# cvg/nice-slam

Measured on AMD Instinct MI355X. Metric: rendered rays/sec (fwd+bwd) per mapping iter, higher is better.
Workload: dtype f32 (f64 sample placement / depth)

## Files before the change

### include/nsr.h

```cpp
#ifndef NSR_H_
#define NSR_H_

#include <stdint.h>

#ifdef __cplusplus
extern "C" {
#endif

#define NSR_VERSION 8

enum { NSR_STAGE_COARSE = 0, NSR_STAGE_MIDDLE = 1, NSR_STAGE_FINE = 2, NSR_STAGE_COLOR = 3 };
enum { NSR_COARSE = 0, NSR_MIDDLE = 1, NSR_FINE = 2, NSR_COLOR = 3 };

#define NSR_MAX_SAMPLES 64

typedef struct nsr_grid {
    const float *feat;
    float *dfeat;
    int32_t Z, Y, X;
    int32_t pad_;
    double lo[3];
    double hi[3];
} nsr_grid;

// ... 43 lines not shown
    const double *d_depth;
    const double *d_var;
    const float *d_rgb;
    const double *depth;
    float *d_rays_o;
    float *d_rays_d;
    float *workspace;
    int64_t workspace_floats;
    int32_t max_blocks;
    int32_t overwrite_dparams;
    void *ev_start;
    void *ev_stop;
    const double *grad_scale;
    int32_t loss_grads_from_forward;
    int32_t pad_;
    void *ev_dx_done;
    void *ev_dw_done;
} nsr_bwd_args;

int nsr_version(void);
const char *nsr_last_error(void);

int64_t nsr_param_count(int slot);
int64_t nsr_packed_count(int slot);
int64_t nsr_acts_floats(int stage, int64_t n_rays, int n_samples_total);

int64_t nsr_bwd_workspace_floats(int stage, int64_t n_rays, int n_samples_total, int max_blocks);

int nsr_pack_params(int slot, const float *params, float *packed, void *stream);

int nsr_render_fwd(const nsr_render_args *a, void *stream);
int nsr_render_bwd(const nsr_render_args *a, const nsr_bwd_args *b, void *stream);

int nsr_eval_points_fwd(const nsr_render_args *a, const double *points, int64_t n_points, float *out, void *stream);

int nsr_get_samples(const int64_t *indices, int64_t n, int32_t H0, int32_t H1, int32_t W0, int32_t W1,
                    int32_t W_full, float fx, float fy, float cx, float cy,
                    const float *c2w, int32_t c2w_stride, const float *depth, const float *color,
                    float *rays_o, float *rays_d, float *out_depth, float *out_color, void *stream);

typedef struct nsr_frame {
    const float *depth;
    const float *color;
    const float *c2w;
    int32_t c2w_stride;
    int32_t pad_;
} nsr_frame;
int nsr_get_samples_window(const int64_t *indices, int32_t K, int64_t n, int32_t H0, int32_t H1, int32_t W0, int32_t W1,
                           int32_t W_full, float fx, float fy, float cx, float cy, const nsr_frame *frames,
                           float *rays_o, float *rays_d, float *out_depth, float *out_color,
                           const double *bound_lo, const double *bound_hi, uint8_t *keep, float *kept_max, void *stream);
int nsr_get_samples_window_draw(int64_t *indices_out, uint64_t *rng_state, int32_t K, int64_t n, int32_t H0, int32_t H1, int32_t W0,
                                int32_t W1, int32_t W_full, float fx, float fy, float cx, float cy, const nsr_frame *frames,
                                float *rays_o, float *rays_d, float *out_depth, float *out_color,
                                const double *bound_lo, const double *bound_hi, uint8_t *keep, float *kept_max, void *stream);
int nsr_get_samples_window_fused(const int64_t *indices, int64_t *indices_out, uint64_t *state, int32_t K, int64_t n, int32_t H0, int32_t H1,
                                 int32_t W0, int32_t W1, int32_t W_full, float fx, float fy, float cx, float cy, const nsr_frame *frames,
                                 float *rays_o, float *rays_d, float *out_depth, float *out_color,
                                 const double *bound_lo, const double *bound_hi, uint8_t *keep, float *header,
                                 float *zero, int64_t zero_floats, void *stream);
int nsr_get_samples_window_sharded(int64_t *indices_out, uint64_t *state, const uint64_t *peer_seeds, int32_t n_peers, int32_t K, int64_t n,
                                   int32_t H0, int32_t H1, int32_t W0, int32_t W1, int32_t W_full, float fx, float fy, float cx, float cy,
                                   const nsr_frame *frames, float *rays_o, float *rays_d, float *out_depth, float *out_color,
                                   const double *bound_lo, const double *bound_hi, uint8_t *keep, float *header,
                                   float *zero, int64_t zero_floats, void *stream);
int nsr_pose_grad(const int64_t *indices, int32_t K, int64_t n, int32_t H0, int32_t H1, int32_t W0, int32_t W1,
// ... 186 lines not shown
```

### nice_slam_amd/_capi.py

```python
from __future__ import annotations

import ctypes as C
import os

import torch

MAX_SAMPLES = 64
ABI_VERSION = 8
STAGE_ID = {"coarse": 0, "middle": 1, "fine": 2, "color": 3}
SLOT_NAMES = ("coarse", "middle", "fine", "color")

_HERE = os.path.dirname(os.path.abspath(__file__))
LIB_PATH = os.environ.get("NSR_LIB_PATH", os.path.join(_HERE, "libnsr.so"))


class NsrGrid(C.Structure):
    _fields_ = [("feat", C.c_void_p), ("dfeat", C.c_void_p),
                ("Z", C.c_int32), ("Y", C.c_int32), ("X", C.c_int32), ("pad_", C.c_int32),
                ("lo", C.c_double * 3), ("hi", C.c_double * 3)]


class NsrDecoder(C.Structure):
    _fields_ = [("params", C.c_void_p), ("packed", C.c_void_p), ("dparams", C.c_void_p)]

# ... 34 lines not shown

class NsrSpan(C.Structure):
    _fields_ = [("ptr", C.c_void_p), ("n", C.c_int64)]


class NsrFrameDesc(C.Structure):
    _fields_ = [("color_h", C.c_int32), ("color_w", C.c_int32), ("depth_h", C.c_int32), ("depth_w", C.c_int32),
                ("depth_type", C.c_int32), ("color_bgr", C.c_int32),
                ("crop_h", C.c_int32), ("crop_w", C.c_int32), ("crop_edge", C.c_int32), ("has_distortion", C.c_int32),
                ("fx", C.c_double), ("fy", C.c_double), ("cx", C.c_double), ("cy", C.c_double),
                ("dist", C.c_double * 5), ("png_depth_scale", C.c_double), ("scale", C.c_double)]


class NsrAdamSpan(C.Structure):
    _fields_ = [("p", C.c_void_p), ("g", C.c_void_p), ("m", C.c_void_p), ("v", C.c_void_p), ("n", C.c_int64), ("step", C.c_void_p),
                ("lr", C.c_float), ("pad_", C.c_int32)]


class NsrAdamGrid(C.Structure):
    _fields_ = [("p", C.c_void_p), ("g", C.c_void_p), ("m", C.c_void_p), ("v", C.c_void_p), ("voxel_mask", C.c_void_p),
                ("n_voxels", C.c_int64), ("step", C.c_void_p), ("lr", C.c_float), ("pad_", C.c_int32)]


SYMBOLS = (
    ("nsr_version", C.c_int, []),
    ("nsr_last_error", C.c_char_p, []),
    ("nsr_param_count", C.c_int64, [C.c_int]),
    ("nsr_packed_count", C.c_int64, [C.c_int]),
    ("nsr_acts_floats", C.c_int64, [C.c_int, C.c_int64, C.c_int]),
    ("nsr_bwd_workspace_floats", C.c_int64, [C.c_int, C.c_int64, C.c_int, C.c_int]),
    ("nsr_pack_params", C.c_int, [C.c_int, C.c_void_p, C.c_void_p, C.c_void_p]),
    ("nsr_render_fwd", C.c_int, [C.POINTER(NsrRenderArgs), C.c_void_p]),
    ("nsr_render_bwd", C.c_int, [C.POINTER(NsrRenderArgs), C.POINTER(NsrBwdArgs), C.c_void_p]),
    ("nsr_eval_points_fwd", C.c_int, [C.POINTER(NsrRenderArgs), C.c_void_p, C.c_int64, C.c_void_p, C.c_void_p]),
    ("nsr_masked_adam", C.c_int, [C.c_void_p, C.c_void_p, C.c_void_p, C.c_void_p, C.c_void_p, C.c_int64,
                                  C.c_float, C.c_float, C.c_float, C.c_float, C.c_float, C.c_void_p]),
    ("nsr_get_samples", C.c_int, [C.c_void_p, C.c_int64, C.c_int32, C.c_int32, C.c_int32, C.c_int32, C.c_int32,
                                  C.c_float, C.c_float, C.c_float, C.c_float, C.c_void_p, C.c_int32,
                                  C.c_void_p, C.c_void_p, C.c_void_p, C.c_void_p, C.c_void_p, C.c_void_p, C.c_void_p]),
    ("nsr_get_samples_window", C.c_int, [C.c_void_p, C.c_int32, C.c_int64, C.c_int32, C.c_int32, C.c_int32, C.c_int32, C.c_int32,
                                         C.c_float, C.c_float, C.c_float, C.c_float, C.POINTER(NsrFrame),
                                         C.c_void_p, C.c_void_p, C.c_void_p, C.c_void_p,
                                         C.POINTER(C.c_double), C.POINTER(C.c_double), C.c_void_p, C.c_void_p, C.c_void_p]),
    ("nsr_get_samples_window_draw", C.c_int, [C.c_void_p, C.c_void_p, C.c_int32, C.c_int64, C.c_int32, C.c_int32, C.c_int32, C.c_int32,
                                              C.c_int32, C.c_float, C.c_float, C.c_float, C.c_float, C.POINTER(NsrFrame),
                                              C.c_void_p, C.c_void_p, C.c_void_p, C.c_void_p,
                                              C.POINTER(C.c_double), C.POINTER(C.c_double), C.c_void_p, C.c_void_p, C.c_void_p]),
    ("nsr_get_samples_window_fused", C.c_int, [C.c_void_p, C.c_void_p, C.c_void_p, C.c_int32, C.c_int64, C.c_int32, C.c_int32, C.c_int32, C.c_int32,
                                               C.c_int32, C.c_float, C.c_float, C.c_float, C.c_float, C.POINTER(NsrFrame),
                                               C.c_void_p, C.c_void_p, C.c_void_p, C.c_void_p,
                                               C.POINTER(C.c_double), C.POINTER(C.c_double), C.c_void_p, C.c_void_p, C.c_void_p, C.c_int64, C.c_void_p]),
    ("nsr_get_samples_window_sharded", C.c_int, [C.c_void_p, C.c_void_p, C.POINTER(C.c_uint64), C.c_int32, C.c_int32, C.c_int64, C.c_int32, C.c_int32,
                                                 C.c_int32, C.c_int32, C.c_int32, C.c_float, C.c_float, C.c_float, C.c_float, C.POINTER(NsrFrame),
                                                 C.c_void_p, C.c_void_p, C.c_void_p, C.c_void_p,
                                                 C.POINTER(C.c_double), C.POINTER(C.c_double), C.c_void_p, C.c_void_p, C.c_void_p, C.c_int64, C.c_void_p]),
    ("nsr_pose_grad", C.c_int, [C.c_void_p, C.c_int32, C.c_int64, C.c_int32, C.c_int32, C.c_int32, C.c_int32,
                                C.c_float, C.c_float, C.c_float, C.c_float, C.c_void_p, C.c_void_p, C.c_void_p, C.c_int32, C.c_void_p]),
    ("nsr_masked_adam_multi", C.c_int, [C.POINTER(NsrAdamGrid), C.c_int32, C.c_double, C.c_double, C.c_double, C.c_int32,
                                        C.c_void_p, C.c_void_p]),
    ("nsr_flat_adam", C.c_int, [C.POINTER(NsrAdamSpan), C.c_int32, C.c_double, C.c_double, C.c_double, C.c_int32, C.c_void_p, C.c_void_p]),
    ("nsr_pack_rows", C.c_int, [C.POINTER(NsrRows), C.c_int32, C.POINTER(NsrSpan), C.c_int32, C.c_void_p, C.c_int32, C.c_void_p]),
    ("nsr_tracking_loss", C.c_int, [C.c_int64, C.c_void_p, C.c_void_p, C.c_void_p, C.c_void_p, C.c_void_p, C.c_void_p,
                                    C.c_int32, C.c_int32, C.c_float, C.c_void_p, C.c_void_p, C.c_void_p, C.c_void_p]),
    ("nsr_camera_from_tensor", C.c_int, [C.c_void_p, C.c_int64, C.c_void_p, C.c_void_p, C.c_void_p, C.c_void_p]),
    ("nsr_aabb_keep", C.c_int, [C.c_void_p, C.c_void_p, C.c_void_p, C.c_int64, C.POINTER(C.c_double), C.POINTER(C.c_double),
                                C.c_void_p, C.c_void_p, C.c_void_p]),
# ... 158 lines not shown
```

### nice_slam_amd/csrc/nsr_api.cpp

```cpp
#include <cmath>
#include <cstdio>
#include <cstdlib>
#include <cstring>
#include <map>
#include <mutex>
#include <string>
#include <utility>

#include "nsr_rt.h"
#include "nsr_kernels.h"
#include "../../nice_slam_amd/csrc/nsr_recon.h"
#include "../../nice_slam_amd/csrc/nsr_bound.h"
#include "../../nice_slam_amd/csrc/nsr_raster.h"
#include "../../nice_slam_amd/csrc/nsr_view.h"
#include "../../nice_slam_amd/csrc/nsr_imgmetrics.h"
#include "../../nice_slam_amd/csrc/nsr_figure.h"
#include "../../nice_slam_amd/csrc/nsr_frame.h"
#include "../../nice_slam_amd/csrc/nsr_pose.h"

namespace {

thread_local std::string g_err;

int fail(const std::string &msg) {
    g_err = msg;
    return 1;
}

constexpr int kMaxTiles = 12;
constexpr int kDefaultBwdBlocks = 256;
constexpr int kLdsLimit = 160 * 1024;
constexpr int kKeyframeBlocks = 256;

#ifndef NSR_TEST_FWD_SMALL
#define NSR_TEST_FWD_SMALL 1
#endif
#ifndef NSR_TEST_HOT_CELLS
#define NSR_TEST_HOT_CELLS 6
#endif
#ifndef NSR_TEST_HOT_SLOTS
#define NSR_TEST_HOT_SLOTS 512
#endif
constexpr bool kFwdSmallBlocks = NSR_TEST_FWD_SMALL != 0;
constexpr int kHotCells = NSR_TEST_HOT_CELLS;
constexpr int kHotSlotCap = NSR_TEST_HOT_SLOTS;
constexpr int kDxFullWeight = 10, kDxLightWeight = 6;
constexpr int kDwWeight = 224;
inline int dw_fine_weight(int stage) { return stage == NSR_STAGE_COLOR ? 240 : 260; }
constexpr int kFinThreads = 1024;
constexpr int kFwdWeight = 10;
inline int fwd_fine_weight(int stage) { return stage == NSR_STAGE_FINE ? 12 : 14; }

inline int round16(int bytes) { return (bytes + 15) & ~15; }

int rays_per_block(int S) {
    const int rb = (kMaxTiles * nsr::kTile) / S;
    return rb < 1 ? 1 : rb;
}

int stage_passes(int stage) { return stage == NSR_STAGE_COARSE ? 1 : 3; }

int max_param_count(int stage) {
    return stage == NSR_STAGE_COARSE ? nsr::param_total(0) : nsr::param_total(2);
}

int bwd_passes(int stage) { return stage == NSR_STAGE_COARSE ? 1 : stage; }

struct SplitLayout {
    long long npts, npad, stride;
    long long o_dy, o_draw, o_pf, o_pd, total;
};
SplitLayout split_layout(int stage, long long n_rays, int S) {
    SplitLayout L;
    const int passes = bwd_passes(stage);
    L.npts = n_rays * S;
    L.npad = (L.npts + nsr::kTile - 1) / nsr::kTile * nsr::kTile;
    L.stride = L.npad * 16;
    L.o_dy = (long long)passes * nsr::kActSlots * L.stride;
    L.o_draw = L.o_dy + (long long)passes * nsr::kDySlots * L.stride;
    L.o_pf = L.o_draw + L.npad * 4;
    L.o_pd = L.o_pf + L.npad * 4;
    L.total = L.o_pd + L.npad * 8;
    return L;
}
// ... 257 lines not shown
extern "C" {

int nsr_version(void) { return NSR_VERSION; }
const char *nsr_last_error(void) { return g_err.c_str(); }

int64_t nsr_param_count(int slot) { return (slot < 0 || slot > 3) ? -1 : nsr::param_total(slot); }
int64_t nsr_packed_count(int slot) { return (slot < 0 || slot > 3) ? -1 : nsr::packed_buf_total(slot); }

int64_t nsr_acts_floats(int stage, int64_t n_rays, int n_samples_total) {
    if (stage < 0 || stage > 3 || n_rays < 0 || n_samples_total < 1 || n_samples_total > NSR_MAX_SAMPLES) return -1;
    return split_layout(stage, n_rays, n_samples_total).total;
}

int64_t nsr_bwd_workspace_floats(int stage, int64_t n_rays, int n_samples_total, int max_blocks) {
    if (stage < 0 || stage > 3 || n_samples_total < 1 || n_samples_total > NSR_MAX_SAMPLES) return -1;
    const SplitGeo G = split_geo(stage, n_rays, n_samples_total, max_blocks);
    const long long split = (long long)bwd_passes(stage) * ((long long)G.nimg * max_param_count(stage) + (long long)G.nb * nsr::kDbPart);
    return (int64_t)split;
}

int nsr_pack_params(int slot, const float *params, float *packed, void *stream) {
    if (slot < 0 || slot > 3) return fail("nsr_pack_params: slot out of range");
    if (!params || !packed) return fail("nsr_pack_params: null pointer");
    const int n = nsr::packed_buf_total(slot), tb = 256, nb = (n + tb - 1) / tb;
    switch (slot) {
        case 0: NSR_LAUNCH(nsr::pack_kernel<0>, dim3(nb), dim3(tb), 0, stream, params, packed); break;
        case 1: NSR_LAUNCH(nsr::pack_kernel<1>, dim3(nb), dim3(tb), 0, stream, params, packed); break;
        case 2: NSR_LAUNCH(nsr::pack_kernel<2>, dim3(nb), dim3(tb), 0, stream, params, packed); break;
        default: NSR_LAUNCH(nsr::pack_kernel<3>, dim3(nb), dim3(tb), 0, stream, params, packed); break;
    }
    return finish("nsr_pack_params");
}

int nsr_render_fwd(const nsr_render_args *a, void *stream) {
    nsr::RenderParams P;
    if (int rc = build_params(a, P, true)) return rc;
#ifdef NSR_TS
    if (const char *e = getenv("NSR_DBG_FWD_PTR")) P.dbg = reinterpret_cast<long long *>(strtoull(e, nullptr, 16));
#endif
    if (!a->depth || !a->var || !a->rgb) return fail("nsr_render_fwd: null output pointer");
    if (P.n_rays == 0) return 0;
    if (a->acts && a->zvals && a->raw) {
        if (P.n_points_total > (1ll << 25) - 16) return fail("nsr_render_fwd: more than 2^25 sample points in one differentiated call (split the ray batch)");
        const int passes = bwd_passes(P.stage), rpb = 4;
        const int w_fine = fwd_fine_weight(P.stage);
        const long long tiles = (P.n_points_total + nsr::kTile - 1) / nsr::kTile;
        const int wsum = passes == 1 ? kFwdWeight : (passes == 2 ? kFwdWeight + w_fine : 2 * kFwdWeight + w_fine);
        long long most = 1;
        P.pass_beg[0] = 0;
        for (int p = 0; p < 3; ++p) {
            int nbp = 0;
            if (p < passes) {
                nbp = (int)((long long)kDefaultBwdBlocks * (p == 1 ? w_fine : kFwdWeight) / wsum);
                if (nbp > tiles) nbp = (int)tiles;
                if (nbp < 1) nbp = 1;
                const long long share = (tiles + nbp - 1) / nbp;
                most = share > most ? share : most;
            }
            P.pass_beg[p + 1] = P.pass_beg[p] + nbp;
        }
        const int waves = (int)(most > nsr::kDxMaxWaves ? nsr::kDxMaxWaves : most);
        const dim3 rgrid((unsigned)((P.n_rays + rpb - 1) / rpb)), rblock(64 * rpb);
        NSR_LAUNCH(nsr::fwd_sample_kernel, rgrid, rblock, rpb * 64 * 8, stream, P);
        int lds = 0;
        const int first = P.stage == NSR_STAGE_COARSE ? NSR_COARSE : NSR_MIDDLE, last = P.stage == NSR_STAGE_COARSE ? NSR_COARSE : P.stage;
        for (int kind = first; kind <= last; ++kind) {
            const int need = (nsr::AUX_FLOATS + nsr::packed_total(kind) + 4) * 4;
            lds = need > lds ? need : lds;
        }
        const dim3 grid(P.pass_beg[3]), block(64 * waves);
#define NSR_FWP(ST, SV)                                                                                      \
    if (int rc = launch_cfg(nsr::render_fwd_pass_kernel<ST, SV>, lds, "nsr_render_fwd(pass)")) return rc;    \
    if (a->ev_pass_start) nsr::rt_record(a->ev_pass_start, stream);                                          \
    NSR_LAUNCH((nsr::render_fwd_pass_kernel<ST, SV>), grid, block, lds, stream, P);                          \
    if (a->ev_pass_stop) nsr::rt_record(a->ev_pass_stop, stream);
        switch (P.stage) {
            case 0: NSR_FWP(0, true) NSR_LAUNCH(nsr::fwd_composite_kernel<0>, rgrid, rblock, rpb * 8, stream, P); break;
            case 1: NSR_FWP(1, true) NSR_LAUNCH(nsr::fwd_composite_kernel<1>, rgrid, rblock, rpb * 8, stream, P); break;
            case 2: NSR_FWP(2, true) NSR_LAUNCH(nsr::fwd_composite_kernel<2>, rgrid, rblock, rpb * 8, stream, P); break;
            default: NSR_FWP(3, true) NSR_LAUNCH(nsr::fwd_composite_kernel<3>, rgrid, rblock, rpb * 8, stream, P); break;
        }
#undef NSR_FWP
        return finish("nsr_render_fwd(split)");
    }
    const int npts = P.rays_per_block * P.S;
    const int lds = fwd_lds_bytes(P.stage, npts);
    const dim3 grid((unsigned)(P.n_groups < (1 << 20) ? P.n_groups : (1 << 20))), block(64 * P.tiles_per_block);
#define NSR_FWD(ST)                                                                               \
    if (int rc = launch_cfg(nsr::render_fwd_kernel<ST>, lds, "nsr_render_fwd")) return rc;         \
    NSR_LAUNCH((nsr::render_fwd_kernel<ST>), grid, block, lds, stream, P);
    P.acts = nullptr;
    switch (P.stage) {
        case 0: NSR_FWD(0) break;
        case 1: NSR_FWD(1) break;
        case 2: NSR_FWD(2) break;
        default: NSR_FWD(3) break;
    }
#undef NSR_FWD
    return finish("nsr_render_fwd");
}

int nsr_render_bwd(const nsr_render_args *a, const nsr_bwd_args *b, void *stream) {
    nsr::RenderParams P;
    if (int rc = build_params(a, P, true, true)) return rc;
    if (!b) return fail("nsr_render_bwd: null backward block");
    if (!a->raw) return fail("nsr_render_bwd: the forward pass must have saved `raw`");
    if (!b->d_depth && !b->d_var && !b->d_rgb) return fail("nsr_render_bwd: no output gradient given");
    if (!b->depth) return fail("nsr_render_bwd: forward depth is required");
    if ((b->d_rays_o == nullptr) != (b->d_rays_d == nullptr)) return fail("nsr_render_bwd: d_rays_o / d_rays_d must be given together");
    if (P.n_rays == 0) return 0;
    P.d_depth = b->d_depth; P.d_var = b->d_var; P.d_rgb = b->d_rgb; P.g_depth = b->depth; P.g_scale = b->grad_scale;
    P.d_rays_o = b->d_rays_o; P.d_rays_d = b->d_rays_d;
#ifdef NSR_TS
    if (const char *e = getenv("NSR_DBG_PTR")) P.dbg = reinterpret_cast<long long *>(strtoull(e, nullptr, 16));
#endif
    const int passes = bwd_passes(P.stage);
    bool any_params = false;
    for (int s = 0; s < 4; ++s) any_params |= P.dec[s].dparams != nullptr;
    P.partial_stride = max_param_count(P.stage);
    if (!P.acts || !a->zvals)
        return fail("nsr_render_bwd: the forward must have been given an activation buffer (nsr_render_args.acts, sized by nsr_acts_floats) and zvals");
    return render_bwd_split(a, b, P, any_params, stream);
}

int nsr_eval_points_fwd(const nsr_render_args *a, const double *points, int64_t n_points, float *out, void *stream) {
    nsr::RenderParams P;
    if (int rc = build_params(a, P, false)) return rc;
    if (n_points < 0 || (n_points > 0 && (!points || !out))) return fail("nsr_eval_points_fwd: bad points / out");
    if (n_points == 0) return 0;
    P.points = points; P.n_points = n_points; P.out_points = out;
    const int waves = kMaxTiles;
    const int wlf = P.stage == NSR_STAGE_COARSE ? nsr::packed_total(0) : (P.stage == NSR_STAGE_MIDDLE ? nsr::packed_total(1) : nsr::packed_total(2));
// ... 1447 lines not shown
```

### nice_slam_amd/csrc/nsr_fwd2.h

```cpp
#pragma once

namespace nsr {

NSR_KERNEL void fwd_sample_kernel(const RenderParams P) {
    double *zs = reinterpret_cast<double *>(lds_base());
    const int lane = tid() & 63, wave = tid() >> 6, nw = nthreads() >> 6;
    const long long ray = (long long)bid_x() * nw + wave;
    const int S = P.S;
    double *zw = zs + wave * 64;
    if (ray >= P.n_rays) return;
    const bool act = lane < S;
    const int k = act ? lane : 0;
    const bool guided = (P.gt_depth != nullptr) && (P.stage != NSR_STAGE_COARSE);
    double z = 0.0;
    {
        const double far_bb = ray_far_bb(P, ray);
        if (!guided) {
            const float tk = P.t_uniform[k];
            const float near_part = 0.01f * (1.f - tk);
            z = (double)near_part + far_bb * (double)tk;
        } else {
            const float gdep = P.gt_depth[ray];
            const float gmax = P.gt_max[0];
            if (k < P.n_samples) {
                const float tk = P.t_uniform[k];
                const double cap = (double)(gmax * 1.2f);
                const double far = tmin(tmax(far_bb, 0.0), cap);
                const float near = gdep * 0.01f;
                z = (double)(near * (1.f - tk)) + far * (double)tk;
            } else {
                const double s = P.t_surface[k - P.n_samples];
                if (gdep > 0.f) {
                    const double e0 = (double)(0.95f * gdep), e1 = (double)(1.05f * gdep);
                    z = e0 * (1.0 - s) + e1 * s;
                } else {
                    z = 0.001 * (1.0 - s) + (double)gmax * s;
                }
            }
        }
    }
    if (P.n_surface > 0 && guided) {
        if (act) zw[lane] = z;
        wave_fence();
// ... 80 lines not shown
                if (active && g == 0) scr[1] = of[0];
            } else {
                const Lvl Lc = make_level(P.grid[NSR_COLOR], px, py, pz);
                const Act<2> ccol = gather_feat(P.grid[NSR_COLOR], Lc, g);
                float oc[4];
                const ActSink sk = act_sink(P, 2, sp, g);
                mlp_xyz_fwd<NSR_COLOR, SAVE>(wl, aux, fx, fy, fz, ccol, lane, oc, &sk);
                if (active && g == 0) { float *rw = P.raw + gp * 4; rw[0] = oc[0]; rw[1] = oc[1]; rw[2] = oc[2]; }
            }
        }
        dbg.stamp(3);
    }
    dbg.stamp(9);
}

template <int STAGE, bool SAVE>
NSR_KERNEL NSR_BOUNDS(768) void render_fwd_pass_kernel(const RenderParams P) {
    const int b = bid_x();
    if (STAGE == NSR_STAGE_COARSE) {
        fwd_pass<NSR_COARSE, SAVE>(P, b, nblk_x());
    } else {
        if (b < P.pass_beg[1]) fwd_pass<NSR_MIDDLE, SAVE>(P, b, P.pass_beg[1]);
        else if (b < P.pass_beg[2]) { if (STAGE >= NSR_STAGE_FINE) fwd_pass<NSR_FINE, SAVE>(P, b - P.pass_beg[1], P.pass_beg[2] - P.pass_beg[1]); }
        else { if (STAGE == NSR_STAGE_COLOR) fwd_pass<NSR_COLOR, SAVE>(P, b - P.pass_beg[2], P.pass_beg[3] - P.pass_beg[2]); }
    }
}

template <int STAGE>
NSR_KERNEL void fwd_composite_kernel(const RenderParams P) {
    double *red = reinterpret_cast<double *>(lds_base());
    const int lane = tid() & 63, wave = tid() >> 6, nw = nthreads() >> 6;
    const long long rayq = (long long)bid_x() * nw + wave;
    const int S = P.S;
    double lterm = 0.0;
    if (rayq < P.n_rays && !ray_live(P, rayq)) {
        if (lane == 0) {
            P.depth[rayq] = 0.0; P.var[rayq] = 0.0;
            P.rgb[rayq * 3 + 0] = 0.f; P.rgb[rayq * 3 + 1] = 0.f; P.rgb[rayq * 3 + 2] = 0.f;
            if (P.loss && P.dl_depth) P.dl_depth[rayq] = 0.0;
            if (P.loss && P.dl_rgb) { P.dl_rgb[rayq * 3 + 0] = 0.f; P.dl_rgb[rayq * 3 + 1] = 0.f; P.dl_rgb[rayq * 3 + 2] = 0.f; }
        }
        if (P.loss && P.dl_depth && lane < S) st4(P.draw + (rayq * S + lane) * 4, F4{0.f, 0.f, 0.f, 0.f});
    } else if (rayq < P.n_rays) {
        const bool act = lane < S;
        const long long gq = rayq * S + (act ? lane : 0);
        const bool kp = !P.loss || !P.keep || P.keep[rayq];
        const float gd = (P.loss && P.loss_depth) ? P.loss_depth[rayq] : 0.f;
        float gtc[3] = {0.f, 0.f, 0.f};
        if (P.loss && STAGE == NSR_STAGE_COLOR && P.gt_color) { gtc[0] = P.gt_color[rayq * 3 + 0]; gtc[1] = P.gt_color[rayq * 3 + 1]; gtc[2] = P.gt_color[rayq * 3 + 2]; }
        double qx = 0.0, qy = 0.0, qz = 0.0, zq = 0.0;
        F4 rw = F4{0.f, 0.f, 0.f, 0.f};
        bool ins = true;
        if (act) {
            const double *pq = P.pd + gq * 4;
            qx = pq[0]; qy = pq[1]; qz = pq[2]; zq = pq[3];
            const float *scr = P.draw + gq * 4;
            float occ = scr[0];
            if (STAGE >= NSR_STAGE_FINE) occ = scr[1] + scr[0];
            if (STAGE == NSR_STAGE_COLOR) { const float *rc = P.raw + gq * 4; rw.x = rc[0]; rw.y = rc[1]; rw.z = rc[2]; }
            ins = (qx > P.blo[0]) && (qx < P.bhi[0]) && (qy > P.blo[1]) && (qy < P.bhi[1]) && (qz > P.blo[2]) && (qz < P.bhi[2]);
            rw.w = ins ? occ : 100.f;
            st4(P.raw + gq * 4, rw);
        }
        const Comp c = comp_weights(rw.w, act, lane);
        const float cr = wave_sum(c.w * rw.x), cg = wave_sum(c.w * rw.y), cb = wave_sum(c.w * rw.z);
        const double depth = wave_sum_d((double)c.w * zq);
// ... 57 lines not shown
```

### nice_slam_amd/csrc/nsr_kernels.h

```cpp
#pragma once
#include "nsr_dev.h"
#include "nsr_layout.h"
#include "../../include/nsr.h"

namespace nsr {

template <int NT>
struct Act { f32x4 t[NT]; };

NSR_DEV f32x4 f4zero() { f32x4 v = {0.f, 0.f, 0.f, 0.f}; return v; }
NSR_DEV f32x4 to_v(F4 a) { f32x4 v = {a.x, a.y, a.z, a.w}; return v; }
NSR_DEV F4 to_F4(f32x4 v) { return F4{v[0], v[1], v[2], v[3]}; }
template <int NT> NSR_DEV void act_zero(Act<NT> &a) {
#pragma unroll
    for (int T = 0; T < NT; ++T) a.t[T] = f4zero();
}

NSR_DEV double tmax(double a, double b) { return (a > b || a != a) ? a : b; }
NSR_DEV double tmin(double a, double b) { return (a < b || a != a) ? a : b; }

struct GridDev {
    const float *feat;
    float *dfeat;
    const unsigned char *gmask;
// ... 25 lines not shown
    double *zvals;
    float *acts;
    int acts_masks_only;
    long long n_points_total;
    long long act_tiles;
    const double *d_depth, *d_var, *g_depth;
    const double *g_scale;
    const float *d_rgb;
    float *d_rays_o, *d_rays_d;
    float *partials;
    int partial_stride;
    const float *loss_depth;
    const float *gt_color;
    const unsigned char *keep;
    double *loss;
    double *dl_depth;
    float *dl_rgb;
    float w_color;
    long long *dbg;
    float *dy;
    float *draw;
    double *pd;
    float *pf;
    float *dbpart;
    int dw_beg[4];
    int dx_beg[4];
    int draw_scaled;
    int skip_masked;
    int lds_grid_floats;
    float hot_z[4];
    int hot_slots;
    unsigned s_magic;
    int pass_beg[4];
    const double *points;
    long long n_points;
    float *out_points;
};

NSR_DEV bool ray_live(const RenderParams &P, long long ray) { return !P.skip_masked || uniform_load_u8(P.keep + ray) != 0u; }
NSR_DEV unsigned ray_of_point(const RenderParams &P, unsigned x) {
    return P.s_magic ? (unsigned)(((unsigned long long)x * P.s_magic) >> 32) : x;
}
NSR_DEV bool tile_live(const RenderParams &P, long long tile) {
    if (!P.skip_masked) return true;
    const unsigned p0 = (unsigned)uniform((int)tile) * kTile, np = (unsigned)P.n_points_total, pe = p0 + kTile < np ? p0 + kTile : np;
    const unsigned r0 = ray_of_point(P, p0), r1 = ray_of_point(P, pe - 1);
    bool live = false;
    for (unsigned r = r0; r <= r1; ++r) live = live || uniform_load_u8(P.keep + r) != 0u;
    return live;
}

template <int KIND>
NSR_DEV float aux_value(const float *__restrict__ flat, int idx) {
    float v = 0.f;
    if (idx < AUX_V) {
        const int i = idx >> 5, o = idx & 31;
        v = flat[bias_off(KIND, i) + o];
    } else if (idx < AUX_WO) {
        if (is_xyz(KIND)) { const int i = (idx - AUX_V) >> 5, o = idx & 31; v = flat[fcb_off(KIND, i) + o]; }
    } else if (idx < AUX_BO) {
        const int n = (idx - AUX_WO) >> 5, k = idx & 31;
        if (n < nout_of(KIND)) v = flat[wo_off(KIND) + n * 32 + k];
    } else if (idx < AUX_BM) {
        const int n = idx - AUX_BO;
        if (n < nout_of(KIND)) v = flat[bo_off(KIND) + n];
    } else if (is_xyz(KIND)) {
// ... 926 lines not shown
    float *rays_o, *rays_d, *out_depth, *out_color;
};

NSR_DEV void pixel_ray(const float *c2w, int stride, float fx, float fy, float cx, float cy, int row, int col, float o[3], float d[3]) {
    const float dx = ((float)col - cx) / fx, dy = -(((float)row - cy) / fy), dzv = -1.f;
#pragma unroll
    for (int a = 0; a < 3; ++a) {
        const float *R = c2w + a * stride;
        d[a] = (dx * R[0] + dy * R[1]) + dzv * R[2];
        o[a] = R[3];
    }
}

NSR_KERNEL void get_samples_kernel(const SampleParams P) {
    const long long t = (long long)bid_x() * nthreads() + tid();
    if (t >= P.n) return;
    const long long idx = P.indices[t];
    const int row = (int)(idx / P.crop_w) + P.H0, col = (int)(idx % P.crop_w) + P.W0;
    const long long pix = (long long)row * P.W_full + col;
    P.out_depth[t] = P.depth[pix];
    P.out_color[t * 3 + 0] = P.color[pix * 3 + 0];
    P.out_color[t * 3 + 1] = P.color[pix * 3 + 1];
    P.out_color[t * 3 + 2] = P.color[pix * 3 + 2];
    const float dx = ((float)col - P.cx) / P.fx, dy = -(((float)row - P.cy) / P.fy), dzv = -1.f;
#pragma unroll
    for (int a = 0; a < 3; ++a) {
        const float *R = P.c2w + a * P.c2w_stride;
        P.rays_d[t * 3 + a] = (dx * R[0] + dy * R[1]) + dzv * R[2];
        P.rays_o[t * 3 + a] = R[3];
    }
}

#define NSR_MAX_WINDOW 32
#define NSR_MAX_PEERS 15
NSR_DEV unsigned philox_word(unsigned c0, unsigned c1, unsigned c2, unsigned c3, unsigned k0, unsigned k1) {
#pragma unroll
    for (int r = 0; r < 10; ++r) {
        const unsigned long long p0 = 0xD2511F53ull * c0, p1 = 0xCD9E8D57ull * c2;
        const unsigned n0 = (unsigned)(p1 >> 32) ^ c1 ^ k0, n1 = (unsigned)p1, n2 = (unsigned)(p0 >> 32) ^ c3 ^ k1, n3 = (unsigned)p0;
        c0 = n0; c1 = n1; c2 = n2; c3 = n3;
        k0 += 0x9E3779B9u; k1 += 0xBB67AE85u;
    }
    return c0;
}

struct WindowParams {
    const long long *indices;
    long long *indices_out;
    unsigned long long *rng;
    unsigned crop_pixels;
    long long n;
    int K, H0, W0, crop_w, W_full;
    float fx, fy, cx, cy;
    const float *depth[NSR_MAX_WINDOW], *color[NSR_MAX_WINDOW], *c2w[NSR_MAX_WINDOW];
    int c2w_stride[NSR_MAX_WINDOW];
    float *rays_o, *rays_d, *out_depth, *out_color;
    double lo[3], hi[3];
    unsigned char *keep;
    float *kept_max;
    float *hdr;
    float *zero;
    long long zero_n;
    int sample_bx;
    int n_peers;
    unsigned long long peer_seed[NSR_MAX_PEERS];
};

NSR_KERNEL void get_samples_window_kernel(const WindowParams P) {
    const int draw_bx = P.sample_bx * (1 + P.n_peers);
    const int peer = bid_x() < draw_bx ? bid_x() / P.sample_bx : 0;
    const bool own = peer == 0;
    const long long i = (long long)(bid_x() - peer * P.sample_bx) * nthreads() + tid();
    const int k = bid_y();
    float vmax = 0.f;
    if (bid_x() >= draw_bx) {
        const long long fb = nblk_x() - draw_bx, chunk = (long long)k * fb + (bid_x() - draw_bx), nchunk = fb * P.K;
        const long long n4 = P.zero_n >> 2;
        for (long long q = chunk * nthreads() + tid(); q < n4; q += nchunk * nthreads()) st4(P.zero + q * 4, F4{0.f, 0.f, 0.f, 0.f});
        if (chunk == 0 && tid() < (int)(P.zero_n & 3)) P.zero[n4 * 4 + tid()] = 0.f;
        return;
    }
    if (i < P.n) {
    const long long t = (long long)k * P.n + i;
    float Rm[3][4];
#pragma unroll
    for (int a = 0; a < 3; ++a) {
        const float *R = P.c2w[k] + a * P.c2w_stride[k];
        Rm[a][0] = R[0]; Rm[a][1] = R[1]; Rm[a][2] = R[2]; Rm[a][3] = R[3];
    }
    long long idx;
    if (P.indices) {
        idx = P.indices[t];
    } else {
        const unsigned long long seed = own ? P.rng[0] : P.peer_seed[peer - 1], call = P.rng[1];
        const unsigned r = philox_word((unsigned)t, (unsigned)(t >> 32), (unsigned)call, (unsigned)(call >> 32), (unsigned)seed, (unsigned)(seed >> 32));
        idx = (long long)(((unsigned long long)r * P.crop_pixels) >> 32);
        if (own) P.indices_out[t] = idx;
    }
    const int row = (int)(idx / P.crop_w) + P.H0, col = (int)(idx % P.crop_w) + P.W0;
    const long long pix = (long long)row * P.W_full + col;
    const float gd = P.depth[k][pix];
    if (own) {
        const float c0 = P.color[k][pix * 3 + 0], c1 = P.color[k][pix * 3 + 1], c2 = P.color[k][pix * 3 + 2];
        P.out_depth[t] = gd;
        P.out_color[t * 3 + 0] = c0;
        P.out_color[t * 3 + 1] = c1;
        P.out_color[t * 3 + 2] = c2;
    }
    const float dx = ((float)col - P.cx) / P.fx, dy = -(((float)row - P.cy) / P.fy), dzv = -1.f;
    double tb = 0.0;
#pragma unroll
    for (int a = 0; a < 3; ++a) {
// ... 911 lines not shown
```

### nice_slam_amd/mapping.py

```python
from __future__ import annotations

import ctypes as C
import os
from typing import List, Optional, Sequence, Tuple

import torch

from . import _capi, engine
from .common import _as_f32c, _require_cuda
from .layout import param_count, stage_slots
from .renderer import RenderCall, _bound6, _gates, _prep_grids, forward_args, render_backward


class WindowSamples:
    __slots__ = ("rays_o", "rays_d", "gt_depth", "gt_color", "keep", "kept_max", "indices", "geom")


def _frames_block(c2ws, depths, colors, dev):
    K = len(depths)
    fr = (_capi.NsrFrame * K)()
    hold = []
    for k in range(K):
        d = _as_f32c(depths[k], dev)
        col = _as_f32c(colors[k], dev)
# ... 32 lines not shown


def _draw_state(dev) -> torch.Tensor:
    key = _dev_key(dev)
    seed = torch.initial_seed() & ((1 << 63) - 1)
    st = _DRAW_STATE.get(key)
    if st is None:
        if _capturing():
            raise RuntimeError("nice_slam_amd: the first in-kernel pixel draw on a device cannot happen under graph capture "
                               "(run one eager iteration first)")
        st = [seed, torch.tensor([seed, 0, 0, 0], dtype=torch.int64, device=dev)]
        _DRAW_STATE[key] = st
    elif st[0] != seed and not _capturing():
        _set_state(st[1], seed)
        st[0] = seed
    return st[1]


def seed_pixel_draws(seed: int, device=None):
    if _capturing():
        raise RuntimeError("nice_slam_amd.seed_pixel_draws: not under graph capture")
    if device is None:
        keys = list(_DRAW_STATE)
    else:
        keys = [_dev_key(torch.device(device))]
    for key in keys:
        st = _DRAW_STATE.get(key)
        if st is None:
            st = _DRAW_STATE[key] = [torch.initial_seed() & ((1 << 63) - 1), torch.zeros(4, dtype=torch.int64, device=torch.device(*key))]
        _set_state(st[1], seed)


DEBUG_PTRS = {} if os.environ.get("NSR_DEBUG_PTRS") == "1" else None


class _Window:
    __slots__ = ("indices", "K", "n", "crop", "intr", "c2ws", "depths", "colors", "bound", "dev", "draw", "state", "peers")

    def __init__(self, crop, n, intr, c2ws, depths, colors, bound, device, indices=None, draw_state=None, peer_seeds=None):
        self.K, self.n, self.dev = len(depths), int(n), torch.device(device)
        self.crop, self.intr = tuple(int(v) for v in crop), tuple(float(v) for v in intr)
        N = self.K * self.n
        self.draw = indices is None and self.dev.type == "cuda"
        if self.draw:
            indices = torch.empty((N,), dtype=torch.int64, device=self.dev)
        elif indices is None:
            H0, H1, W0, W1, _ = self.crop
            indices, draw_state = torch.randint((H1 - H0) * (W1 - W0), (N,), device=self.dev), None
        else:
            indices = indices.to(self.dev).reshape(-1).contiguous()
        self.indices, self.state = indices, draw_state
        self.peers = list(peer_seeds) if (self.draw and peer_seeds) else None
        self.c2ws = [c if isinstance(c, torch.Tensor) else torch.as_tensor(c) for c in c2ws]
        self.depths, self.colors, self.bound = list(depths), list(colors), bound


def _launch_window(win: _Window, frames, rays, kmax_ptr, fused=None):
    E = engine.on(win.dev)
    o, d, gd, gc, keep = rays
    common = (win.K, win.n, *win.crop, *win.intr, frames, o.data_ptr(), d.data_ptr(), gd.data_ptr(), gc.data_ptr(),
              *_bound_arrays(win.bound), keep.data_ptr())
    draw, win.draw = win.draw, False
    state = (win.state if win.state is not None else _draw_state(win.dev)) if (draw or fused is not None) else None
    ind = win.indices.data_ptr()
    if fused is None and draw:
        E.call("nsr_get_samples_window_draw", ind, state.data_ptr(), *common, kmax_ptr)
# ... 65 lines not shown
    @staticmethod
    def _forward_impl(ctx, renderer, decoders, stage, win, w_color, sharder, out, track, *tensors):
        K, N, dev = win.K, win.K * win.n, win.dev
        E = engine.on(dev)
        slots = stage_slots(stage)
        grids = dict(zip(slots, tensors[K:]))
        guided = stage != "coarse"
        S = renderer.N_samples + (renderer.N_surface if guided else 0)
        need = ctx.needs_input_grad[8:]
        need_pose = any(need[:K])
        need_grid = need[K:K + len(slots)]
        need_par = need[K + len(slots):K + 2 * len(slots)]
        need_bwd = need_pose or any(need_grid) or any(need_par)
        n_grad = 0
        if need_bwd:
            n_grad = sum(grids[s].numel() for s, nd in zip(slots, need_grid) if nd) + (6 * N if need_pose else 0) + \
                sum(param_count(s) for s, nd in zip(slots, need_par) if nd)
        n_pose = 16 * K if need_pose else 0
        fuse_fill = N > 0
        if fuse_fill and not win.draw and win.state is None and _capturing() and _dev_key(dev) not in _DRAW_STATE:
            fuse_fill = False
        Z = (torch.empty if fuse_fill else torch.zeros)((4 + n_grad + n_pose,), dtype=torch.float32, device=dev)
        loss = Z[:2].view(torch.float64)
        kmax = Z[2:3]
        frames, hold = _frames_block(win.c2ws, win.depths, win.colors, dev)
        n64 = 3 * N + N * S
        nf32 = N * S * 4 + 6 * N
        n_s = _ray_buffer(N)
        FS = torch.empty((n64 + (nf32 + 1) // 2 + (n_s + 1) // 2,), dtype=torch.float64, device=dev)
        F = FS[:n64 + (nf32 + 1) // 2]
        sbuf = FS[n64 + (nf32 + 1) // 2:].view(torch.float32)[:n_s]
        rays = _ray_buffer(N, sbuf)
        rays_o, rays_d, gt_depth, gt_color, keep = rays
        _launch_window(win, frames, rays, kmax.data_ptr(), fused=(Z[:4], Z[4:]) if fuse_fill else None)
        if sharder is not None and not (fuse_fill and win.peers):
            sharder.reduce_max(kmax)
        f32 = F[n64:].view(torch.float32)
        depth, var, dl_depth, zvals = F[:N], F[N:2 * N], F[2 * N:3 * N], F[3 * N:n64].view(N, S)
        raw, rgb, dl_rgb = f32[:N * S * 4].view(N, S, 4), f32[N * S * 4:N * S * 4 + 3 * N].view(N, 3), f32[N * S * 4 + 3 * N:N * S * 4 + 6 * N].view(N, 3)
        call = RenderCall(renderer, decoders, stage, grids, rays_o, rays_d, gt_depth, hook=None if sharder is None else sharder.collect)
        acts = forward_args(call, renderer.N_surface if guided else 0, kmax, (depth, var, rgb, raw, zvals),
                            [not g_ for g_ in need_par] if need_bwd else None)
        a = call.args
        if track is None:
            a.gt_color, a.loss, a.w_color = gt_color.data_ptr(), loss.data_ptr(), float(w_color)
            a.dl_depth, a.dl_rgb = dl_depth.data_ptr(), dl_rgb.data_ptr()
        a.keep = keep.data_ptr()
        a.skip_masked = 1 if (renderer.skip_masked_rays and need_bwd) else 0
        if need_bwd and renderer.profile_fwd_events is not None:
            a.ev_pass_start, a.ev_pass_stop = renderer.profile_fwd_events(stage)
        if DEBUG_PTRS is not None:
            DEBUG_PTRS[stage] = {"Z": Z.data_ptr(), "Z_bytes": 4 * Z.numel(), "FS": FS.data_ptr(), "acts": None if acts is None else acts.data_ptr(),
                                 "acts_bytes": None if acts is None else 4 * acts.numel(), "grids": {s: grids[s].data_ptr() for s in slots}}
        if need_bwd and acts is None:
            raise _capi.NsrError("nice_slam_amd: the activation buffer of a %d-ray fused iteration does not fit (Renderer."
                                 "max_saved_activation_bytes / free device memory); use smaller batches or render_batch_ray" % N)
        E.call("nsr_render_fwd", C.byref(a))
        if track is not None:
            E.call("nsr_tracking_loss", N, gt_depth.data_ptr(), gt_color.data_ptr(), keep.data_ptr(), depth.data_ptr(), var.data_ptr(),
                   rgb.data_ptr(), int(track[0]), int(track[1]), float(w_color), loss.data_ptr(), dl_depth.data_ptr(), dl_rgb.data_ptr())
        if out is not None:
            out.update(rays_o=rays_o, rays_d=rays_d, gt_depth=gt_depth, gt_color=gt_color, keep=keep, kept_max=kmax, depth=depth,
                       uncertainty=var, color=rgb, indices=win.indices)
        ctx.state = None
        if need_bwd:
            call.hold += [F, sbuf, Z, hold, acts]
            st = ctx.state = _LossState()
            st.call, st.win, st.need, st.sharder = call, win, (need_pose, need_pose, need_grid, need_par), sharder
            st.dl_depth, st.dl_rgb = dl_depth, dl_rgb if (stage == "color" and (track is None or track[1])) else None
            st.zero, st.pose_buf = Z[4:], Z[4 + n_grad:4 + n_grad + n_pose].view(K, 4, 4) if need_pose else None
            st.loss, st.loss32 = loss, Z[3:4]
            st.from_forward = track is None
        return loss[0]

    @staticmethod
    @torch.autograd.function.once_differentiable
    def backward(ctx, g_loss):
        with _capi.on_device(g_loss.device):
            st = ctx.state
            if st is None:
                raise RuntimeError("nice_slam_amd: backward through mapping_loss / tracking_loss a second time is not supported "
                                   "(the saved buffers are released after the first backward)")
            gs = g_loss.detach().to(device=st.dl_depth.device, dtype=torch.float64).reshape(1)
            d_o, d_d, d_grids = render_backward(st.call, st.need, st.dl_depth, None, st.dl_rgb, zero_buf=st.zero, grad_scale=gs,
                                                loss_grads_from_forward=st.from_forward)
            win = st.win
            gp, pose_base = pose_grads(win, d_o, d_d, out=st.pose_buf) if st.need[0] else ([None] * win.K, None)
            if st.sharder is not None:
                st.loss32.copy_(st.loss.to(torch.float32))
                st.sharder.exchange([("grid_" + s_, g) for s_, g in zip(st.call.slots, d_grids) if g is not None], pose_base, st.loss32)
# ... 50 lines not shown
```

Before: 4.736 million.

## Split gradient-buffer zero fill across window, sample and composite kernels

```diff
diff --git a/include/nsr.h b/include/nsr.h
--- a/include/nsr.h
+++ b/include/nsr.h
@@ -99,6 +99,10 @@
 int nsr_render_fwd(const nsr_render_args *a, void *stream);
 int nsr_render_bwd(const nsr_render_args *a, const nsr_bwd_args *b, void *stream);
 
+int nsr_fill_shares(int64_t zero_floats, const int32_t *weights, int64_t *shares);
+int nsr_render_fwd_fill(const nsr_render_args *a, float *fill_sample, int64_t fill_sample_floats, float *fill_composite,
+                        int64_t fill_composite_floats, void *stream);
+
 int nsr_eval_points_fwd(const nsr_render_args *a, const double *points, int64_t n_points, float *out, void *stream);
 
 int nsr_get_samples(const int64_t *indices, int64_t n, int32_t H0, int32_t H1, int32_t W0, int32_t W1,
diff --git a/nice_slam_amd/_capi.py b/nice_slam_amd/_capi.py
--- a/nice_slam_amd/_capi.py
+++ b/nice_slam_amd/_capi.py
@@ -90,6 +90,8 @@
     ("nsr_pack_params", C.c_int, [C.c_int, C.c_void_p, C.c_void_p, C.c_void_p]),
     ("nsr_render_fwd", C.c_int, [C.POINTER(NsrRenderArgs), C.c_void_p]),
     ("nsr_render_bwd", C.c_int, [C.POINTER(NsrRenderArgs), C.POINTER(NsrBwdArgs), C.c_void_p]),
+    ("nsr_fill_shares", C.c_int, [C.c_int64, C.POINTER(C.c_int32), C.POINTER(C.c_int64)]),
+    ("nsr_render_fwd_fill", C.c_int, [C.POINTER(NsrRenderArgs), C.c_void_p, C.c_int64, C.c_void_p, C.c_int64, C.c_void_p]),
     ("nsr_eval_points_fwd", C.c_int, [C.POINTER(NsrRenderArgs), C.c_void_p, C.c_int64, C.c_void_p, C.c_void_p]),
     ("nsr_masked_adam", C.c_int, [C.c_void_p, C.c_void_p, C.c_void_p, C.c_void_p, C.c_void_p, C.c_int64,
                                   C.c_float, C.c_float, C.c_float, C.c_float, C.c_float, C.c_void_p]),
diff --git a/nice_slam_amd/csrc/nsr_api.cpp b/nice_slam_amd/csrc/nsr_api.cpp
--- a/nice_slam_amd/csrc/nsr_api.cpp
+++ b/nice_slam_amd/csrc/nsr_api.cpp
@@ -50,6 +50,13 @@
 constexpr int kFinThreads = 1024;
 constexpr int kFwdWeight = 10;
 inline int fwd_fine_weight(int stage) { return stage == NSR_STAGE_FINE ? 12 : 14; }
+
+constexpr int kFillShare[3] = {6, 6, 8};
+constexpr long long kFillSplitMin = 2ll << 20;
+inline long long fill_blocks(long long n) {
+    const long long want = (n * 4 + 32767) / 32768;
+    return want > 2048 ? 2048 : want;
+}
 
 inline int round16(int bytes) { return (bytes + 15) & ~15; }
 
@@ -373,9 +380,41 @@
     return finish("nsr_pack_params");
 }
 
-int nsr_render_fwd(const nsr_render_args *a, void *stream) {
+int nsr_fill_shares(int64_t zero_floats, const int32_t *weights, int64_t *shares) {
+    if (zero_floats < 0 || !shares) return fail("nsr_fill_shares: bad arguments");
+    const int32_t whole[3] = {1, 0, 0};
+    const int32_t *w = weights ? weights : (zero_floats < kFillSplitMin ? whole : kFillShare);
+    long long wsum = 0;
+    int last = -1;
+    for (int i = 0; i < 3; ++i) {
+        if (w[i] < 0 || w[i] > (1 << 20)) return fail("nsr_fill_shares: weights must be in [0, 2^20]");
+        wsum += w[i];
+        if (w[i]) last = i;
+    }
+    if (last < 0) return fail("nsr_fill_shares: all weights are zero");
+    const long long n4 = zero_floats >> 2;
+    long long beg = 0, cum = 0;
+    for (int i = 0; i < 3; ++i) {
+        cum += w[i];
+        const long long end = i >= last ? zero_floats : 4 * ((n4 / wsum) * cum + (n4 % wsum) * cum / wsum);
+        shares[i] = w[i] ? end - beg : 0;
+        beg += shares[i];
+    }
+    return 0;
+}
+
+}
+namespace {
+int render_fwd(const nsr_render_args *a, float *const fill[2], const int64_t fill_n[2], void *stream) {
     nsr::RenderParams P;
     if (int rc = build_params(a, P, true)) return rc;
+    const bool fills = fill_n[0] > 0 || fill_n[1] > 0;
+    for (int i = 0; i < 2; ++i) {
+        if (fill_n[i] < 0 || (fill_n[i] > 0 && (!fill[i] || (reinterpret_cast<uintptr_t>(fill[i]) & 15))))
+            return fail("nsr_render_fwd_fill: a fill span must be 16-byte aligned");
+    }
+    if (fills && !(P.n_rays > 0 && a->acts && a->zvals && a->raw))
+        return fail("nsr_render_fwd_fill: fill spans need the three-launch forward (acts, zvals and raw given, n_rays >= 1): they would stay unwritten");
 #ifdef NSR_TS
     if (const char *e = getenv("NSR_DBG_FWD_PTR")) P.dbg = reinterpret_cast<long long *>(strtoull(e, nullptr, 16));
 #endif
@@ -401,8 +440,11 @@
             P.pass_beg[p + 1] = P.pass_beg[p] + nbp;
         }
         const int waves = (int)(most > nsr::kDxMaxWaves ? nsr::kDxMaxWaves : most);
-        const dim3 rgrid((unsigned)((P.n_rays + rpb - 1) / rpb)), rblock(64 * rpb);
-        NSR_LAUNCH(nsr::fwd_sample_kernel, rgrid, rblock, rpb * 64 * 8, stream, P);
+        const long long rbx = (P.n_rays + rpb - 1) / rpb;
+        P.ray_bx = (int)rbx;
+        for (int i = 0; i < 2; ++i) { P.fill_z[i] = fill[i]; P.fill_n[i] = fill_n[i]; }
+        const dim3 sgrid((unsigned)(rbx + fill_blocks(fill_n[0]))), rgrid((unsigned)(rbx + fill_blocks(fill_n[1]))), rblock(64 * rpb);
+        NSR_LAUNCH(nsr::fwd_sample_kernel, sgrid, rblock, rpb * 64 * 8, stream, P);
         int lds = 0;
         const int first = P.stage == NSR_STAGE_COARSE ? NSR_COARSE : NSR_MIDDLE, last = P.stage == NSR_STAGE_COARSE ? NSR_COARSE : P.stage;
         for (int kind = first; kind <= last; ++kind) {
@@ -439,6 +481,21 @@
     }
 #undef NSR_FWD
     return finish("nsr_render_fwd");
+}
+}
+extern "C" {
+
+int nsr_render_fwd(const nsr_render_args *a, void *stream) {
+    float *const none[2] = {nullptr, nullptr};
+    const int64_t zero[2] = {0, 0};
+    return render_fwd(a, none, zero, stream);
+}
+
+int nsr_render_fwd_fill(const nsr_render_args *a, float *fill_sample, int64_t fill_sample_floats, float *fill_composite,
+                        int64_t fill_composite_floats, void *stream) {
+    float *const fill[2] = {fill_sample, fill_composite};
+    const int64_t n[2] = {fill_sample_floats, fill_composite_floats};
+    return render_fwd(a, fill, n, stream);
 }
 
 int nsr_render_bwd(const nsr_render_args *a, const nsr_bwd_args *b, void *stream) {
diff --git a/nice_slam_amd/csrc/nsr_fwd2.h b/nice_slam_amd/csrc/nsr_fwd2.h
--- a/nice_slam_amd/csrc/nsr_fwd2.h
+++ b/nice_slam_amd/csrc/nsr_fwd2.h
@@ -8,7 +8,10 @@
     const long long ray = (long long)bid_x() * nw + wave;
     const int S = P.S;
     double *zw = zs + wave * 64;
-    if (ray >= P.n_rays) return;
+    if (ray >= P.n_rays) {
+        if (bid_x() >= P.ray_bx) zero_fill_chunk(P.fill_z[0], P.fill_n[0], bid_x() - P.ray_bx, nblk_x() - P.ray_bx);
+        return;
+    }
     const bool act = lane < S;
     const int k = act ? lane : 0;
     const bool guided = (P.gt_depth != nullptr) && (P.stage != NSR_STAGE_COARSE);
@@ -155,6 +158,10 @@
     const int lane = tid() & 63, wave = tid() >> 6, nw = nthreads() >> 6;
     const long long rayq = (long long)bid_x() * nw + wave;
     const int S = P.S;
+    if ((long long)bid_x() * nw >= P.n_rays) {
+        zero_fill_chunk(P.fill_z[1], P.fill_n[1], bid_x() - P.ray_bx, nblk_x() - P.ray_bx);
+        return;
+    }
     double lterm = 0.0;
     if (rayq < P.n_rays && !ray_live(P, rayq)) {
         if (lane == 0) {
diff --git a/nice_slam_amd/csrc/nsr_kernels.h b/nice_slam_amd/csrc/nsr_kernels.h
--- a/nice_slam_amd/csrc/nsr_kernels.h
+++ b/nice_slam_amd/csrc/nsr_kernels.h
@@ -81,6 +81,9 @@
     int hot_slots;
     unsigned s_magic;
     int pass_beg[4];
+    float *fill_z[2];
+    long long fill_n[2];
+    int ray_bx;
     const double *points;
     long long n_points;
     float *out_points;
@@ -1073,6 +1076,20 @@
 }
 
 #define NSR_MAX_WINDOW 32
+NSR_DEV void st4_zero_through(float *p) {
+#if defined(__AMDGCN__)
+    typedef float v4f __attribute__((ext_vector_type(4)));
+    const v4f zero = {0.f, 0.f, 0.f, 0.f};
+    asm volatile("global_store_dwordx4 %0, %1, off sc1\n\ts_nop 1" ::"v"(p), "v"(zero) : "memory");
+#else
+    st4(p, F4{0.f, 0.f, 0.f, 0.f});
+#endif
+}
+NSR_DEV void zero_fill_chunk(float *z, long long n, long long chunk, long long nchunk) {
+    const long long n4 = n >> 2;
+    for (long long q = chunk * nthreads() + tid(); q < n4; q += nchunk * nthreads()) st4_zero_through(z + q * 4);
+    if (chunk == 0 && tid() < (int)(n & 3)) z[n4 * 4 + tid()] = 0.f;
+}
 #define NSR_MAX_PEERS 15
 NSR_DEV unsigned philox_word(unsigned c0, unsigned c1, unsigned c2, unsigned c3, unsigned k0, unsigned k1) {
 #pragma unroll
@@ -1115,10 +1132,8 @@
     const int k = bid_y();
     float vmax = 0.f;
     if (bid_x() >= draw_bx) {
-        const long long fb = nblk_x() - draw_bx, chunk = (long long)k * fb + (bid_x() - draw_bx), nchunk = fb * P.K;
-        const long long n4 = P.zero_n >> 2;
-        for (long long q = chunk * nthreads() + tid(); q < n4; q += nchunk * nthreads()) st4(P.zero + q * 4, F4{0.f, 0.f, 0.f, 0.f});
-        if (chunk == 0 && tid() < (int)(P.zero_n & 3)) P.zero[n4 * 4 + tid()] = 0.f;
+        const long long fb = nblk_x() - draw_bx;
+        zero_fill_chunk(P.zero, P.zero_n, (long long)k * fb + (bid_x() - draw_bx), fb * P.K);
         return;
     }
     if (i < P.n) {
diff --git a/nice_slam_amd/mapping.py b/nice_slam_amd/mapping.py
--- a/nice_slam_amd/mapping.py
+++ b/nice_slam_amd/mapping.py
@@ -88,6 +88,22 @@
 
 
 DEBUG_PTRS = {} if os.environ.get("NSR_DEBUG_PTRS") == "1" else None
+
+
+FILL_WEIGHTS = None
+_FILL_SHARES = {}
+
+
+def _fill_shares(lib, n: int):
+    key = (n, None if FILL_WEIGHTS is None else tuple(int(w) for w in FILL_WEIGHTS))
+    sh = _FILL_SHARES.get(key)
+    if sh is None:
+        out = (C.c_int64 * 3)()
+        lib.check(lib.nsr_fill_shares(n, None if key[1] is None else (C.c_int32 * 3)(*key[1]), out), "nsr_fill_shares")
+        if len(_FILL_SHARES) > 64:
+            _FILL_SHARES.clear()
+        sh = _FILL_SHARES[key] = tuple(int(v) for v in out)
+    return sh
 
 
 class _Window:
@@ -219,7 +235,8 @@
         sbuf = FS[n64 + (nf32 + 1) // 2:].view(torch.float32)[:n_s]
         rays = _ray_buffer(N, sbuf)
         rays_o, rays_d, gt_depth, gt_color, keep = rays
-        _launch_window(win, frames, rays, kmax.data_ptr(), fused=(Z[:4], Z[4:]) if fuse_fill else None)
+        n_a, n_b, n_c = _fill_shares(E.lib, Z.numel() - 4) if fuse_fill else (0, 0, 0)
+        _launch_window(win, frames, rays, kmax.data_ptr(), fused=(Z[:4], Z[4:4 + n_a]) if fuse_fill else None)
         if sharder is not None and not (fuse_fill and win.peers):
             sharder.reduce_max(kmax)
         f32 = F[n64:].view(torch.float32)
@@ -242,7 +259,11 @@
         if need_bwd and acts is None:
             raise _capi.NsrError("nice_slam_amd: the activation buffer of a %d-ray fused iteration does not fit (Renderer."
                                  "max_saved_activation_bytes / free device memory); use smaller batches or render_batch_ray" % N)
-        E.call("nsr_render_fwd", C.byref(a))
+        if n_b or n_c:
+            zp = Z.data_ptr() + 4 * (4 + n_a)
+            E.call("nsr_render_fwd_fill", C.byref(a), zp if n_b else None, n_b, zp + 4 * n_b if n_c else None, n_c)
+        else:
+            E.call("nsr_render_fwd", C.byref(a))
         if track is not None:
             E.call("nsr_tracking_loss", N, gt_depth.data_ptr(), gt_color.data_ptr(), keep.data_ptr(), depth.data_ptr(), var.data_ptr(),
                    rgb.data_ptr(), int(track[0]), int(track[1]), float(w_color), loss.data_ptr(), dl_depth.data_ptr(), dl_rgb.data_ptr())
```

Result: slower. 4.652 million (-1.8%).
